# tabahi/WebSpeechAnalyzer

Measured on AMD Instinct MI355X. Metric: 53-feat frames/sec, higher is better.
Workload: dtype f32 front end / f64 tracker; 1 GPU; 1024 clips x 10 s @16 kHz mono per GPU, 1024-pt FFT, 25 ms hop, Segment Features (level 5); parallelism=1 GPU, batches_in_flight=6, streams=3

## Files before the change

### webspeechanalyzer_amd/csrc/tracker.hip

```cpp
#include <type_traits>
#include "wsa_internal.hpp"
#include "jsmath_device.hpp"
#include "wave_ops.hpp"
#include "tracker_score.hpp"
#include "tracker_features.hpp"

#ifdef WSA_TUNING
#define WSA_TUNE(bits_) (p.dbg & (bits_))
#else
#define WSA_TUNE(bits_) false
#endif

namespace wsa {

constexpr int MAXC = 64;
constexpr int AC_MAX = 320;
constexpr int PAIR_AC = 64;
constexpr int PAIR_GSZ = 4384;
constexpr int QUAD_AC = 38;
constexpr int QUAD_GSZ = 2496;
constexpr int AC_FAST = 140;

struct Ws {
    int32_t *tr_len, *tr_slot, *tr_rank;
// ... 108 lines not shown
        t.item++;
        const uint2 e = p.order[idx];
        t.clip = e.x; t.seg = e.y;
    }
    else if (DEAL == DEAL_GROUPS) {
        t.total = p.counters[p.order_cnt];
        const uint32_t npairs = (t.total + (uint32_t)NGR - 1u) / (uint32_t)NGR, W_ = gridDim.x, r = t.item;
        if ((uint64_t)r * W_ >= npairs) return SPAN_DONE;
        t.item++;
        t.group = (uint64_t)r * W_ + ((r & 1u) ? W_ - 1u - blockIdx.x : blockIdx.x);
        if (t.group >= npairs) return SPAN_SKIP;
    }
    else if (p.order) {
        const uint32_t total = p.counters[p.order_cnt], W_ = gridDim.x, r = t.item;
        if ((uint64_t)r * W_ >= total) return SPAN_DONE;
        t.item++;
        const uint64_t idx = (uint64_t)r * W_ + ((r & 1u) ? W_ - 1u - blockIdx.x : blockIdx.x);
        if (idx >= total) return SPAN_SKIP;
        const uint2 e = p.order[idx];
        t.clip = e.x; t.seg = e.y;
    } else {
        t.seg = t.item / p.n_clips; t.clip = t.item - t.seg * p.n_clips;
        if (t.seg >= p.counters[0]) return SPAN_DONE;
        t.item += gridDim.x;
        if (t.seg >= p.seg_count[t.clip]) return SPAN_SKIP;
    }
    return SPAN_TAKE;
}

}
#include "tracker_finalize.hpp"
#include "tracker_one.hpp"
#include "tracker_group.hpp"
namespace wsa {

template <int AC, bool RAW>
__device__ __forceinline__ void one_span_body(const TrParams& p) {
    const OneLds<AC> L = carve_lds<AC>();
    const int lane = threadIdx.x;
    SpanState sp;
    sp.W = carve_ws(p.ws + (uint64_t)blockIdx.x * p.ws_stride, p.tcap, p.pcap, p.fcap, RAW ? p.pcap : 0, nullptr);
    sp.gen = 0; sp.aev_stride = p.fcap + 2;
    for (int d = lane; d < p.fcap + 2; d += 64) sp.W.d_gen[d] = 0;
    wsync();
    SpanTurn t{p.order ? 0u : blockIdx.x};
    for (;;) {
        const int turn = next_span<DEAL_SPANS>(p, t);
        if (turn == SPAN_DONE) break;
        if (turn == SPAN_SKIP) continue;
        sp.begin(p, t.clip, (int)t.seg); sp.load_segment(p, true); sp.gen++;
        const unsigned long long tk0 = (WSA_TUNE(DBG_CYCLES)) ? __builtin_readcyclecounter() : 0ull;
        track_span<AC, RAW>(p, sp, L, lane);
        const unsigned long long tk1 = (WSA_TUNE(DBG_CYCLES)) ? __builtin_readcyclecounter() : 0ull;
        finish_span<AC, RAW, false>(p, sp, L, lane);
        trace_span_cycles(p, sp, lane, tk0, tk1);
        if (sp.overflow && lane == 0) atomicOr(&p.shared[1], sp.act_overflow && AC < AC_MAX ? 2u : 1u);
        wsync();
    }
}
template <int AC, bool RAW>
__device__ __forceinline__ void stream_body(const TrParams& p) {
    const OneLds<AC> L = carve_lds<AC>();
    const int lane = threadIdx.x;
    SpanState sp;
    sp.W = carve_ws(p.ws + (uint64_t)blockIdx.x * p.ws_stride, p.tcap, p.pcap, p.fcap, RAW ? p.pcap : 0, nullptr);
    sp.aev_stride = p.fcap + 2;
    wsync();
    sp.begin(p, blockIdx.x, 0);
    const unsigned long long tk0 = (WSA_TUNE(DBG_CYCLES)) ? __builtin_readcyclecounter() : 0ull;
    track_stream<AC, RAW>(p, sp, L, lane);
    trace_span_cycles(p, sp, lane, tk0, tk0);
    if (sp.overflow && lane == 0) atomicOr(&p.shared[1], 1u);
    wsync();
}
template <int AC, int GW, int SPLIT>
__device__ __forceinline__ void group_body(const TrParams& p) {
    const OneLds<AC, GW == 16> L = carve_lds<AC, GW == 16>();
    const int lane = threadIdx.x;
    SpanState sp;
    sp.gen = 0; sp.aev_stride = p.fcap + 2;
    if (!SPLIT) for (int h = 0; h < 2; h++) {
        const Ws Wh = carve_ws(p.ws + ((uint64_t)blockIdx.x * 2 + h) * p.ws_stride, p.tcap, p.pcap, p.fcap, 0, nullptr);
        for (int d = lane; d < p.fcap + 2; d += 64) Wh.d_gen[d] = 0;
    }
    wsync();
    SpanTurn t{p.order ? 0u : blockIdx.x};
    for (;;) {
        const int turn = next_span<DEAL_GROUPS, 64 / GW>(p, t);
        if (turn == SPAN_DONE) break;
        if (turn == SPAN_SKIP) continue;
        sp.gen++;
        track_group<AC, GW, SPLIT>(p, sp, L, lane, t);
    }
}
template <int AC>
__device__ __forceinline__ void finalize_body(const TrParams& p) {
    const OneLds<AC> L = carve_lds<AC>();
    const int lane = threadIdx.x;
    SpanState sp;
    wsync();
    SpanTurn t{p.order ? 0u : blockIdx.x};
    for (;;) {
        if (next_span<DEAL_FINALIZE>(p, t) == SPAN_DONE) break;
        sp.begin(p, t.clip, (int)t.seg); sp.load_segment(p, true);
        finalize_from_header<AC>(p, sp, L, lane);
    }
}

__global__ __launch_bounds__(64) __attribute__((amdgpu_waves_per_eu(4, 4))) void tracker_kernel_fast(TrParams p) { one_span_body<AC_FAST, false>(p); }
__global__ __launch_bounds__(64) __attribute__((amdgpu_waves_per_eu(3, 4))) void tracker_kernel_pair(TrParams p) {
    __builtin_amdgcn_s_setprio(3);
    group_body<AC_FAST, 32, 0>(p);
}
__global__ __launch_bounds__(64) __attribute__((amdgpu_waves_per_eu(4, 4))) void tracker_kernel_pair_acc(TrParams p) {
    __builtin_amdgcn_s_setprio(3);
    group_body<AC_FAST, 32, 1>(p);
}
__global__ __launch_bounds__(64) __attribute__((amdgpu_waves_per_eu(4, 4))) void tracker_kernel_quad_acc(TrParams p) {
    __builtin_amdgcn_s_setprio(3);
    group_body<AC_FAST, 16, 1>(p);
}
__global__ __launch_bounds__(64) __attribute__((amdgpu_waves_per_eu(4, 4))) void tracker_kernel_finalize(TrParams p) {
    __builtin_amdgcn_s_setprio(3);
    finalize_body<AC_FAST>(p);
}
__global__ __launch_bounds__(64) void tracker_kernel_full(TrParams p) { one_span_body<AC_MAX, false>(p); }
__global__ __launch_bounds__(64) void tracker_kernel_raw(TrParams p) { one_span_body<AC_MAX, true>(p); }
__global__ __launch_bounds__(64) void tracker_kernel_stream(TrParams p) { stream_body<AC_MAX, false>(p); }
__global__ __launch_bounds__(64) void tracker_kernel_stream_raw(TrParams p) { stream_body<AC_MAX, true>(p); }

constexpr int ORDER_T = 256;
__global__ __launch_bounds__(ORDER_T) void span_order_kernel(const uint32_t* hist, const uint2* key, const uint32_t* seg_count, uint32_t n_clips, int seg_cap, uint2* order, uint32_t* counters) {
    __shared__ uint32_t offs[SPAN_BUCKETS], part[ORDER_T];
    const int tid = threadIdx.x;
    constexpr int PER = SPAN_BUCKETS / ORDER_T;
    uint32_t mine[PER], sum = 0;
#pragma unroll
    for (int q = 0; q < PER; q++) { mine[q] = hist[tid * PER + q]; sum += mine[q]; }
    part[tid] = sum;
    __syncthreads();
    for (int d = 1; d < ORDER_T; d <<= 1) {
        const uint32_t add = tid >= d ? part[tid - d] : 0u;
        __syncthreads();
        part[tid] += add;
        __syncthreads();
    }
    uint32_t run = part[tid] - sum;
#pragma unroll
    for (int q = 0; q < PER; q++) { offs[tid * PER + q] = run; run += mine[q]; }
    if (blockIdx.x == 0 && tid == ORDER_T - 1) counters[1] = part[tid];
    __syncthreads();
    const uint32_t clip = blockIdx.x * ORDER_T + tid;
    if (clip >= n_clips) return;
    const uint32_t ns = seg_count[clip];
    for (uint32_t k = 0; k < ns; k++) {
        const uint2 e = key[(uint64_t)clip * seg_cap + k];
        order[offs[e.x] + e.y] = make_uint2(clip, k);
    }
}

void launch_span_order(const TrParams& p, uint32_t* span_hist, const uint2* span_key, uint2* order, uint32_t* counters, hipStream_t s) {
    if (p.n_clips == 0) return;
    hipLaunchKernelGGL(span_order_kernel, dim3((p.n_clips + ORDER_T - 1) / ORDER_T), dim3(ORDER_T), 0, s, span_hist, span_key, p.seg_count, p.n_clips, p.seg_cap, order, counters);
}

void launch_tracker_stream(const TrParams& p, uint32_t n_streams, hipStream_t s) {
    if (n_streams == 0) return;
    static_assert(AC_MAX == TR_ACT_MAX, "the streams' saved active table is sized for the full variant");
    if (p.level == 3) hipLaunchKernelGGL(tracker_kernel_stream_raw, dim3(n_streams), dim3(64), 0, s, p);
    else hipLaunchKernelGGL(tracker_kernel_stream, dim3(n_streams), dim3(64), 0, s, p);
}

void launch_tracker(const TrParams& p, int n_waves, bool full_table, bool pair, hipStream_t s) {
    if (n_waves <= 0) return;
    if (p.level == 3) hipLaunchKernelGGL(tracker_kernel_raw, dim3(n_waves), dim3(64), 0, s, p);
    else if (full_table) hipLaunchKernelGGL(tracker_kernel_full, dim3(n_waves), dim3(64), 0, s, p);
    else if (pair && p.order && p.redo && (!p.trace || (p.dbg & DBG_CYCLES))) {
        if (p.pool && p.span_hdr) {
            if (p.quad) hipLaunchKernelGGL(tracker_kernel_quad_acc, dim3(p.quad_waves > 0 ? p.quad_waves : n_waves), dim3(64), 0, s, p);
            else hipLaunchKernelGGL(tracker_kernel_pair_acc, dim3(n_waves), dim3(64), 0, s, p);
            hipLaunchKernelGGL(tracker_kernel_finalize, dim3(p.fin_waves > 0 ? p.fin_waves : 2 * n_waves), dim3(64), 0, s, p);
        }
        else hipLaunchKernelGGL(tracker_kernel_pair, dim3(n_waves), dim3(64), 0, s, p);
        TrParams r = p; r.order = p.redo; r.order_cnt = 2; r.pool = nullptr; r.span_hdr = nullptr;
        const int redo_waves = p.quad ? 1024 : 128;
        hipLaunchKernelGGL(tracker_kernel_fast, dim3(n_waves < redo_waves ? n_waves : redo_waves), dim3(64), 0, s, r);
    }
    else hipLaunchKernelGGL(tracker_kernel_fast, dim3(n_waves), dim3(64), 0, s, p);
}

__global__ void compact_count_kernel(CompactParams p) {
    const uint32_t c = blockIdx.x * blockDim.x + threadIdx.x;
    if (c >= p.n_clips) return;
    const uint32_t ns = p.seg_count[c];
    const int32_t* sg = p.seg_i + (uint64_t)c * p.seg_cap * 8;
    uint32_t r = 0;
    for (uint32_t k = 0; k < ns; k++) if (sg[8 * k + SEG_FLAG] >= 0) r += (uint32_t)sg[8 * k + SEG_NROWS];
    p.clip_row_off[c] = r;
}
constexpr int CSCAN_T = 1024;
template <bool COUNT>
__global__ __launch_bounds__(CSCAN_T) void compact_scan_kernel(CompactParams p) {
    __shared__ uint32_t s_rows[CSCAN_T], s_segs[CSCAN_T];
    const int tid = threadIdx.x;
    const uint32_t per = (p.n_clips + CSCAN_T - 1) / CSCAN_T;
    const uint32_t c0 = min(p.n_clips, tid * per), c1 = min(p.n_clips, c0 + per);
    uint32_t rs = 0, ss = 0;
    for (uint32_t c = c0; c < c1; c++) {
        if (COUNT) {
            const uint32_t ns = p.seg_count[c];
            const int32_t* sg = p.seg_i + (uint64_t)c * p.seg_cap * 8;
            uint32_t r = 0;
            for (uint32_t k = 0; k < ns; k++) if (sg[8 * k + SEG_FLAG] >= 0) r += (uint32_t)sg[8 * k + SEG_NROWS];
            p.clip_row_off[c] = r;
        }
        ss += p.seg_count[c]; rs += p.clip_row_off[c];
    }
    s_rows[tid] = rs; s_segs[tid] = ss;
    __syncthreads();
    for (int d = 1; d < CSCAN_T; d <<= 1) {
        const uint32_t ar_ = tid >= d ? s_rows[tid - d] : 0u, as_ = tid >= d ? s_segs[tid - d] : 0u;
        __syncthreads();
        s_rows[tid] += ar_; s_segs[tid] += as_;
        __syncthreads();
    }
    if (tid == CSCAN_T - 1) {
        p.totals[0] = s_rows[tid]; p.totals[1] = s_segs[tid];
        p.clip_row_off[p.n_clips] = s_rows[tid]; p.clip_seg_off[p.n_clips] = s_segs[tid];
    }
    uint32_t ar = s_rows[tid] - rs, as = s_segs[tid] - ss;
    for (uint32_t c = c0; c < c1; c++) {
        const uint32_t r = p.clip_row_off[c];
        p.clip_row_off[c] = ar; p.clip_seg_off[c] = as; as += p.seg_count[c]; ar += r;
    }
// ... 90 lines not shown
```

### webspeechanalyzer_amd/csrc/tracker_finalize.hpp

```cpp
#pragma once

namespace wsa {

__device__ __forceinline__ long long take_rows(const TrParams& p, SpanState& sp, int lane, int n) {
    uint32_t r0 = 0;
    if (lane == 0) r0 = atomicAdd(&p.clip_rows[sp.clip], (uint32_t)n);
    r0 = (uint32_t)read_lane_i32((int)r0, 0);
    if ((uint64_t)r0 + (uint32_t)n > p.row_cap) { sp.overflow = true; return -1; }
    return (long long)sp.clip * p.row_cap + r0;
}
template <typename Clear>
__device__ __forceinline__ int qualify_tracks(const Ws& W, int n_tr, int lane, double* qmb, int32_t* qt, Clear&& clear) {
    int nq = 0;
    for (int base = 0; base < n_tr; base += 64) {
        const int t = base + lane;
        bool q = false; double mb = 0;
        if (t < n_tr) {
            clear(t);
            const int tl = W.tr_len[t]; const double sb = W.tr_sumEbin[t], se = W.tr_sumE[t];
            if (tl >= 2) { mb = sb / se; q = mb >= 7; }
        }
        const uint64_t mask = __ballot(q);
        if (q) { const int pos = nq + __popcll(mask & lanemask_lt(lane)); qmb[pos] = mb; qt[pos] = t; }
        nq += __popcll(mask);
// ... 40 lines not shown
template <typename Part>
__device__ __forceinline__ bool files_past_the_end(const SpanState& sp, int lane, bool by_index, Part&& takes_part) {
    bool bad = false;
    for (int base = sp.len; base <= (by_index ? sp.c_ci + 1 : -1); base += 64) {
        const int d = base + lane;
        if (d <= sp.c_ci + 1 && sp.W.d_gen[d] == sp.gen)
            for (int q = sp.W.d_p0[d]; q < sp.W.d_p1[d]; q++) if (takes_part(q)) bad = true;
    }
    if (sp.stale_d >= sp.len && lane == 0)
        for (int q = 0; q < sp.stale_p1; q++) if (takes_part(q)) bad = true;
    return bad;
}
template <typename Key, typename KeyOf, typename Point>
__device__ __forceinline__ void straighten_select(const TrParams& p, const SpanState& sp, int lane, float* fr, float* smv, KeyOf&& key_of, Point&& point) {
    for (int base = 0; base < ((WSA_TUNE(DBG_NO_STRAIGHTEN)) ? 0 : sp.len); base += 64) {
        const int d = base + lane;
        if (d < sp.len) {
            float f9[9];
#pragma unroll
            for (int q = 0; q < 9; q++) f9[q] = 0.f;
            float sm = 0.f;
            const int a1 = (sp.stale_d == d) ? sp.stale_p1 : 0;
            const int dg = sp.W.d_gen[d], dp0 = sp.W.d_p0[d], dp1 = sp.W.d_p1[d];
            const bool has_main = dg == sp.gen;
            const int b0 = has_main ? dp0 : 0, b1 = has_main ? dp1 : 0;
            Key last_key = -1;
            for (;;) {
                Key best_key = sizeof(Key) == 4 ? (Key)0x7fffffff : (Key)0x7fffffffffffffffLL; int best_q = -1;
                for (int part = 0; part < 2; part++) {
                    const int q0 = part ? b0 : 0, q1 = part ? b1 : a1;
                    for (int q = q0; q < q1; q++) {
                        const Key key = key_of(q);
                        if (key > last_key && key < best_key) { best_key = key; best_q = q; }
                    }
                }
                if (best_q < 0) break;
                last_key = best_key;
                int l; double f, wd, E;
                point(best_q, l, f, wd, E);
                const float cur = l == 0 ? f9[0] : (l == 1 ? f9[3] : f9[6]);
                if ((double)cur > sp.floor_ && (double)cur < f && l < 2) l++;
                const float ff = (float)f, Ef = (float)E, wf = (float)wd;
                if (l == 0) { f9[0] = ff; f9[1] = Ef; f9[2] = wf; }
                else if (l == 1) { f9[3] = ff; f9[4] = Ef; f9[5] = wf; }
                else { f9[6] = ff; f9[7] = Ef; f9[8] = wf; }
                sm = (float)((double)sm + E);
            }
#pragma unroll
            for (int q = 0; q < 9; q++) fr[9 * d + q] = f9[q];
            smv[d] = sm;
        }
    }
}
template <bool LANES, typename Feat>
__device__ __forceinline__ void write_rows(const TrParams& p, SpanState& sp, int lane, const float* fr, const float* smv, Feat&& features) {
    if (p.formants && (p.level == 4 || p.level == 10)) {
        for (int q = lane; q < 9 * sp.len; q += 64) { const int d = q / 9; p.formants[((uint64_t)sp.foff + (((uint32_t)sp.start + (uint32_t)d) & p.ring_mask)) * 9 + (uint32_t)(q - 9 * d)] = fr[q]; }
        if (p.sums) { for (int q = lane; q < sp.len; q += 64) p.sums[(uint64_t)sp.foff + (((uint32_t)sp.start + (uint32_t)q) & p.ring_mask)] = smv[q]; }
    }
    double accS, accC; sp.totals(accS, accC);
    const double cs = accC / accS;
    const double lg_ctx = jsm::log10(sp.ctx_max);
    if (p.level == 4 || p.level == 5) {
        const long long r0 = take_rows(p, sp, lane, 1);
        if (r0 < 0) return;
        double* x = p.row_feat + (uint64_t)r0 * WSA_NFEAT;
        if (WSA_TUNE(DBG_CYCLES)) sp.ph[2] = __builtin_readcyclecounter();
        if (p.level == 5) {
            if (!(WSA_TUNE(DBG_NO_FEATURES))) features(fr, sp.len, x);
            if (WSA_TUNE(DBG_CYCLES)) sp.ph[3] = __builtin_readcyclecounter();
            if (lane == 0) { x[0] = sp.len; x[1] = sqrt((double)sp.len); x[2] = cs; x[3] = lg_ctx; x[4] = sp.floor_; }
        } else if (lane < WSA_NFEAT) x[lane] = 0;
        if (lane == 0) {
            int32_t* m = p.row_meta + (uint64_t)r0 * 8;
            m[0] = (int32_t)sp.clip; m[1] = 0; m[2] = 0; m[3] = 0; m[4] = sp.my_seg; m[5] = 0; m[6] = sp.start; m[7] = sp.len;
            sp.sg[SEG_FLAG] = 1; sp.sg[SEG_NROWS] = 1; sp.sg[SEG_ROW0] = (int32_t)r0;
        }
        return;
    }
    int nsyl = 0, my_si = 0, my_sl = 0;
    {
        int si = -1, cc = 0, uu = 0;
        for (int base = 0; base < sp.len; base += 64) {
            const int dd = base + lane;
            const float smq = dd < sp.len ? smv[dd] : 0.f;
            const int lim = min(64, sp.len - base);
            for (int j = 0; j < lim; j++) {
                const int e2 = base + j;
                const double v = __builtin_bit_cast(float, read_lane_i32(__builtin_bit_cast(int, smq), j));
                if (v > sp.floor_) { cc = 0; uu++; if (si < 0) si = e2; } else cc++;
                if ((uu > 20 && cc > 0) || (uu > 10 && cc > 1) || (uu > 0 && cc > 4) || (e2 >= sp.len - 1 && uu > 4)) {
                    const int t = e2 - cc;
                    if (t - si > 1) {
                        if (LANES && nsyl < 64) { if (lane == nsyl) { my_si = si; my_sl = t - si; } }
                        else if (lane == 0) { sp.W.q_idx[2 * nsyl] = si; sp.W.q_idx[2 * nsyl + 1] = t - si; }
                        nsyl++;
                        si = -1; uu = 0;
                    }
                }
            }
        }
    }
    wsync();
    long long r0 = 0;
    if (nsyl > 0) { r0 = take_rows(p, sp, lane, nsyl); if (r0 < 0) return; }
    for (int k = 0; k < nsyl; k++) {
        const int si = LANES && k < 64 ? read_lane_i32(my_si, k) : sp.W.q_idx[2 * k], sl = LANES && k < 64 ? read_lane_i32(my_sl, k) : sp.W.q_idx[2 * k + 1];
        double* x = p.row_feat + (uint64_t)(r0 + k) * WSA_NFEAT;
        if (p.level == 13) {
            if (!(WSA_TUNE(DBG_NO_FEATURES))) features(fr + 9 * si, sl, x);
            if (lane == 0) { x[0] = sl; x[1] = sqrt((double)sl); x[2] = cs; x[3] = lg_ctx; x[4] = sp.floor_; }
        } else if (lane < WSA_NFEAT) x[lane] = 0;
        if (lane == 0) {
            int32_t* m = p.row_meta + (uint64_t)(r0 + k) * 8;
            m[0] = (int32_t)sp.clip; m[1] = 0; m[2] = si; m[3] = sl; m[4] = sp.my_seg; m[5] = k; m[6] = sp.start + si; m[7] = sl;
        }
    }
    if (lane == 0) { sp.sg[SEG_FLAG] = nsyl > 0 ? 1 : 0; sp.sg[SEG_NROWS] = nsyl; sp.sg[SEG_ROW0] = (int32_t)r0; }
}
template <int AC, bool G>
__device__ __forceinline__ bool finalize_lds(const TrParams& p, SpanState& sp, const OneLds<AC>& L, int lane) {
    constexpr int BIG = OneLds<AC>::BYTES;
    const int off_u = (int)align16((size_t)2 * sp.n_tr);
    const int rank_bytes = 16 * sp.n_tr, fr_bytes = G ? 0 : (int)align16((size_t)40 * sp.len);
    const int off_pt = off_u + fr_bytes;
    const bool pe_lds = !G && off_pt + 12 * sp.n_pt <= BIG;
    const int ppb = pe_lds ? 12 : 4;
    if (sp.n_tr > 8000 || sp.n_pt > 60000 || off_u + rank_bytes > BIG || off_pt + ppb * sp.n_pt > BIG || off_pt + FEAT_SCRATCH * 8 > BIG) return false;
    int16_t* const trk_key = reinterpret_cast<int16_t*>(L.big);
    double* const qmb = reinterpret_cast<double*>(L.big + off_u);
    int32_t* const qt = reinterpret_cast<int32_t*>(L.big + off_u + 8 * sp.n_tr);
    int32_t* const srt = qt + sp.n_tr;
    float* const fr = G ? sp.W.fr : reinterpret_cast<float*>(L.big + off_u);
    float* const smv = G ? sp.W.sm1 : fr + 9 * sp.len;
    double* const pE = reinterpret_cast<double*>(L.big + off_pt);
    uint32_t* const pkb = reinterpret_cast<uint32_t*>(L.big + off_pt + (pe_lds ? 8 * sp.n_pt : 0));
    auto energy_of = [&](int q) __attribute__((always_inline)) -> double { return pe_lds ? pE[q] : reinterpret_cast<const double*>(sp.W.pt + q)[1]; };
    if (WSA_TUNE(DBG_CYCLES)) sp.ph[0] = sp.ph[1] = sp.ph[2] = sp.ph[3] = __builtin_readcyclecounter();
    const int nq = qualify_tracks(sp.W, sp.n_tr, lane, qmb, qt, [&](int t) __attribute__((always_inline)) { trk_key[t] = -1; });
    wsync();
    rank_tracks(nq, qmb, lane, [&](int rank, int qi) __attribute__((always_inline)) { srt[rank] = qi; });
    wsync();
    const int n_part = assign_slots(nq, qmb, qt, srt, lane, [&](int t, int key) __attribute__((always_inline)) { trk_key[t] = (int16_t)key; });
    wsync();
    const int off_tbl = (int)align16((size_t)off_pt + (size_t)ppb * (size_t)sp.n_pt);
    const int tbl_bytes = 4 * (sp.len + 1) + 2 * (sp.len + 1) * n_part;
    const bool use_tbl = !G && n_part <= 32 && sp.c_ci + 1 < 0x7fff && sp.stale_d < 0x7fff && off_tbl + tbl_bytes <= BIG && !(p.dbg & DBG_SELECT_LOOP);
    uint32_t* const tblm = reinterpret_cast<uint32_t*>(L.big + off_tbl);
    uint16_t* const tbl = reinterpret_cast<uint16_t*>(tblm + sp.len + 1);
    if (use_tbl) for (int q = lane; q <= sp.len; q += 64) tblm[q] = 0u;
    wsync();
    bool bad = false;
    {
        int4 nxt4 = lane < sp.n_pt ? sp.W.pt[lane] : make_int4(0, 0, 0, 0);
        for (int q = lane; q < sp.n_pt; q += 64) {
            const int4 rec4 = nxt4;
            if (q + 64 < sp.n_pt) nxt4 = sp.W.pt[q + 64];
            const int key = trk_key[rec4.x];
            if (pe_lds) pE[q] = __hiloint2double(rec4.w, rec4.z);
            pkb[q] = ((uint32_t)rec4.y & 0x1ffffu) | ((key < 0 ? 0x7fffu : (uint32_t)key) << 17);
            if (use_tbl && key >= 0) {
                const int d = (int)((uint32_t)rec4.y >> 17);
                if (d >= sp.len) bad = true;
                else {
                    const int row = (q < sp.stale_p1 && sp.stale_d >= 0) ? sp.len : d;
                    tbl[row * n_part + (key >> 2)] = (uint16_t)(q + 1);
                    atomicOr(&tblm[row], 1u << (key >> 2));
                }
            }
        }
    }
    wsync();
    if (WSA_TUNE(DBG_CYCLES)) sp.ph[0] = __builtin_readcyclecounter();
    if (files_past_the_end(sp, lane, !use_tbl, [&](int q) __attribute__((always_inline)) { return (pkb[q] >> 17) != 0x7fffu; })) bad = true;
    if (__ballot(bad) != 0ull) { if (lane == 0) { sp.sg[SEG_FLAG] = -1; sp.sg[SEG_NROWS] = 0; } return true; }
    if (use_tbl) {
        const uint32_t stale_m = tblm[sp.len];
        float thr_f;
        { const double t0 = sp.floor_ < 0 ? 0.0 : floor(sp.floor_) + 1.0; thr_f = (float)(t0 > 256.0 ? 256.0 : t0); }
        for (int base = 0; base < ((WSA_TUNE(DBG_NO_STRAIGHTEN)) ? 0 : sp.len); base += 64) {
            const int d = base + lane;
            float* const row = fr + 9 * (d < sp.len ? d : 0);
            if (d < sp.len) {
#pragma unroll
                for (int q = 0; q < 9; q++) row[q] = 0.f;
            }
            float sm = 0.f;
            auto apply = [&](int q) __attribute__((always_inline)) {
                const uint32_t w = pkb[q];
                int l = (int)((w >> 17) & 3u);
                const double E = energy_of(q);
                const float ff = (float)(w & 0xffu), cur = row[3 * l];
                if (cur >= thr_f && cur < ff && l < 2) l++;
                row[3 * l] = ff; row[3 * l + 1] = (float)E; row[3 * l + 2] = (float)((w >> 8) & 0x1ffu);
                sm = (float)((double)sm + E);
            };
            const uint32_t m_main = d < sp.len ? tblm[d] : 0u, m_st = (d < sp.len && d == sp.stale_d) ? stale_m : 0u;
            uint32_t mm = m_main | m_st;
            while (mm) {
                const int r = __ffs((int)mm) - 1; mm &= mm - 1u;
                if ((m_st >> r) & 1u) apply((int)tbl[sp.len * n_part + r] - 1);
                if ((m_main >> r) & 1u) apply((int)tbl[d * n_part + r] - 1);
            }
            if (d < sp.len) smv[d] = sm;
        }
    } else
    straighten_select<int>(p, sp, lane, fr, smv,
        [&](int q) __attribute__((always_inline)) -> int { const uint32_t w = pkb[q]; return (w >> 17) == 0x7fffu ? -1 : (int)(((w >> 19) << 16) | (uint32_t)q); },
        [&](int q, int& l, double& f, double& wd, double& E) __attribute__((always_inline)) {
            const uint32_t w = pkb[q];
            l = (int)((w >> 17) & 3u); f = w & 0xffu; wd = (w >> 8) & 0x1ffu; E = energy_of(q);
        });
    wsync();
    if (WSA_TUNE(DBG_CYCLES)) sp.ph[1] = __builtin_readcyclecounter();
    double* const red = reinterpret_cast<double*>(L.big + off_pt);
    write_rows<true>(p, sp, lane, fr, smv, [&](const float* f, int n, double* x) __attribute__((always_inline)) {
        formant_features_lds(f, n, sp.ctx_max, x, lane, red, !G && n <= 15 && !(p.dbg & DBG_NO_PACKED_COLUMNS), G || (p.dbg & DBG_EVENTS_BLOCK) != 0);
    });
    return true;
}
template <int AC>
__device__ __forceinline__ void finalize_generic(const TrParams& p, SpanState& sp, const OneLds<AC>& L, int lane) {
    constexpr int FRCAP = OneLds<AC>::FRCAP;
    if (WSA_TUNE(DBG_CYCLES)) sp.ph[0] = sp.ph[1] = sp.ph[2] = sp.ph[3] = __builtin_readcyclecounter();
    const int nq = qualify_tracks(sp.W, sp.n_tr, lane, sp.W.q_mb, sp.W.q_idx, [&](int t) __attribute__((always_inline)) { sp.W.tr_slot[t] = -1; });
    wsync();
    const bool q_lds = nq <= AC;
    double* qmb = sp.W.q_mb; int32_t* qidx = sp.W.q_idx; int32_t* sorted = sp.W.sorted;
    if (q_lds) {
        for (int qi = lane; qi < nq; qi += 64) { L.f_qmb[qi] = sp.W.q_mb[qi]; L.f_qidx[qi] = sp.W.q_idx[qi]; }
        qmb = L.f_qmb; qidx = L.f_qidx; sorted = L.f_sorted;
        wsync();
    }
    rank_tracks(nq, qmb, lane, [&](int rank, int qi) __attribute__((always_inline)) { sorted[rank] = qi; });
    wsync();
    assign_slots(nq, qmb, qidx, sorted, lane, [&](int t, int key) __attribute__((always_inline)) { sp.W.tr_slot[t] = key; });
    wsync();
    {
        int t_nxt = lane < sp.n_pt ? sp.W.pt[lane].x : 0;
        for (int q = lane; q < sp.n_pt; q += 64) {
            const int t = t_nxt;
            if (q + 64 < sp.n_pt) t_nxt = sp.W.pt[q + 64].x;
            sp.W.pt_key[q] = sp.W.tr_slot[t];
        }
    }
    wsync();
    if (WSA_TUNE(DBG_CYCLES)) sp.ph[0] = __builtin_readcyclecounter();
    if (__ballot(files_past_the_end(sp, lane, true, [&](int q) __attribute__((always_inline)) { return sp.W.pt_key[q] >= 0; })) != 0ull) { if (lane == 0) { sp.sg[SEG_FLAG] = -1; sp.sg[SEG_NROWS] = 0; } return; }
    float* const fr = sp.len <= FRCAP ? L.f_fr : sp.W.fr;
    float* const smv_ = sp.len <= FRCAP ? L.f_sm : sp.W.sm1;
    auto features = [&](const float* f, int a, double* x) __attribute__((always_inline)) {
        if (sp.len > FRCAP && a <= FEAT_LDS_MAX) formant_features_lds(f, a, sp.ctx_max, x, lane, reinterpret_cast<double*>(L.big), false, true);
        else formant_features_wave(f, a, sp.ctx_max, x, sp.W.Aev, sp.aev_stride, lane);
    };
    straighten_select<long long>(p, sp, lane, fr, smv_,
        [&](int q) __attribute__((always_inline)) -> long long { const int pk = sp.W.pt_key[q]; return pk < 0 ? -1LL : (long long)(pk >> 2) * (long long)(p.pcap + 1) + q; },
        [&](int q, int& l, double& f, double& wd, double& E) __attribute__((always_inline)) {
            l = sp.W.pt_key[q] & 3;
            const int4 rec4 = sp.W.pt[q];
            f = rec4.y & 0xff; wd = (rec4.y >> 8) & 0x1ff; E = __hiloint2double(rec4.w, rec4.z);
        });
    wsync();
    if (WSA_TUNE(DBG_CYCLES)) sp.ph[1] = __builtin_readcyclecounter();
    write_rows<false>(p, sp, lane, fr, smv_, features);
}
__device__ __forceinline__ void export_raw_tracks(const TrParams& p, SpanState& sp, int lane, bool ring) {
    const int nq = qualify_tracks(sp.W, sp.n_tr, lane, sp.W.q_mb, sp.W.q_idx, [](int) __attribute__((always_inline)) {});
    wsync();
    const uint64_t pbase = (uint64_t)sp.foff * MAXC;
    const uint64_t pmask = ring ? (uint64_t)(p.ring_mask + 1u) * MAXC - 1ull : ~0ull;
    const uint64_t poff = (ring ? (uint64_t)((uint32_t)sp.sg[SEG_FBEGIN] & p.ring_mask) : (uint64_t)sp.f_begin) * MAXC;
    const uint64_t pool0 = pbase + poff;
    auto slot = [&](uint64_t q) __attribute__((always_inline)) -> uint64_t { return pbase + ((poff + q) & pmask); };
    rank_tracks(nq, sp.W.q_mb, lane, [&](int rank, int qi) __attribute__((always_inline)) { p.trk_rank[slot((uint64_t)rank)] = sp.W.q_idx[qi]; });
    for (int q = lane; q < sp.n_pt; q += 64) { int4 v = sp.W.pt[q]; v.y &= 0x1ffff; p.trk_pts[2 * slot((uint64_t)q)] = v; p.trk_pts[2 * slot((uint64_t)q) + 1] = sp.W.ptx[q]; }
    if (lane == 0) {
        int32_t* ts = p.trk_seg + ((uint64_t)sp.clip * p.seg_cap + sp.my_seg) * 4;
        ts[0] = (int32_t)(pool0 & 0xffffffffu); ts[1] = sp.n_pt; ts[2] = nq; ts[3] = (int32_t)(pool0 >> 32);
    }
}
template <int AC, bool RAW, bool THIRD>
__device__ __forceinline__ void finish_span(const TrParams& p, SpanState& sp, const OneLds<AC>& L, int lane, bool ring = false) {
    for (int j = lane; j < sp.n_act; j += 64) { const int gi = L.a_gid[j]; sp.W.tr_len[gi] = L.a_len[j]; sp.W.tr_sumE[gi] = L.a_sumE[j]; sp.W.tr_sumEbin[gi] = L.a_sumEbin[j]; }
    wsync();
    if constexpr (RAW) export_raw_tracks(p, sp, lane, ring);
    else if (!(WSA_TUNE(DBG_NO_FINALIZE))) {
        if (!(p.dbg & DBG_GENERIC_FINALIZE)) {
            if (finalize_lds<AC, false>(p, sp, L, lane)) return;
            if constexpr (THIRD) { if (!(p.dbg & DBG_NO_THIRD_FORM) && finalize_lds<AC, true>(p, sp, L, lane)) return; }
        }
        finalize_generic<AC>(p, sp, L, lane);
    }
}
template <int AC>
__device__ __forceinline__ void finalize_from_header(const TrParams& p, SpanState& sp, const OneLds<AC>& L, int lane) {
    const double* hd = p.span_hdr + ((uint64_t)sp.clip * p.seg_cap + (uint32_t)sp.my_seg) * 8;
    const double h0 = hd[0], h1 = hd[1], h2 = hd[2], h3 = hd[3], h4 = hd[4], h5 = hd[5], h6 = hd[6];
    const int flag = (int)h6;
    if (flag == 0) return;
    if (flag & 2) { if (lane == 0) atomicOr(&p.shared[1], 1u); return; }
    const int F = (int)(sp.f_end - sp.f_begin);
    sp.W = carve_ws(p.pool + (uint64_t)(sp.foff + sp.f_begin) * p.pool_bpf, MAXC * F, MAXC * F, F, 0, nullptr);
    sp.aev_stride = F + 2;
    sp.n_tr = (int)h0; sp.n_pt = (int)h1; sp.n_act = 0; sp.stale_d = (int)h2; sp.stale_p1 = (int)h3;
    sp.accG = h4; sp.accL = lane == 0 ? h5 : 0.0;
    sp.gen = 1;
    const unsigned long long tf0 = WSA_TUNE(DBG_CYCLES) ? __builtin_readcyclecounter() : 0ull;
    finish_span<AC, false, true>(p, sp, L, lane);
    if (WSA_TUNE(DBG_CYCLES) && lane == 0 && p.trace) {
        double* tr = p.trace + (uint64_t)atomicAdd(&p.shared[0], 1u) * 12;
        tr[0] = 0; tr[1] = (double)(__builtin_readcyclecounter() - tf0); tr[2] = sp.len; tr[3] = F; tr[4] = sp.n_tr; tr[5] = sp.n_pt; tr[6] = blockIdx.x;
        tr[7] = (double)(sp.ph[0] - tf0); tr[8] = (double)(sp.ph[1] - sp.ph[0]); tr[9] = (double)(sp.ph[2] - sp.ph[1]); tr[10] = (double)(sp.ph[3] - sp.ph[2]);
    }
    if (sp.overflow && lane == 0) atomicOr(&p.shared[1], 1u);
    wsync();
}

}
```

### webspeechanalyzer_amd/csrc/tracker_group.hpp

```cpp
#pragma once

namespace wsa {

template <int GW>
struct GroupLds {
    static constexpr int ACG = GW == 32 ? PAIR_AC : QUAD_AC, NGR = 64 / GW, GSZ = GW == 32 ? PAIR_GSZ : QUAD_GSZ;
    static_assert(GSZ % 16 == 0 && GSZ >= ACG * 48 + GW * 40 + 24 && (ACG * 24) % 8 == 0 && (ACG * 48 + GW * 20) % 8 == 0, "group layout fits its share of the block");
    double *t_vel, *t_sumE, *t_sumEbin; uint32_t* t_mmask; int32_t *t_lf, *t_len, *t_gid; uint32_t *t_bins, *t_amp;
    uint32_t *q_pk, *q_amp, *q_plo, *q_phi, *q_hi;
    unsigned long long* q_best; int32_t *q_asg, *q_prj, *q_pro;
    uint32_t* q_map;
    __device__ __forceinline__ GroupLds(unsigned char* big, int g) {
        unsigned char* const gb = big + g * GSZ;
        t_vel = reinterpret_cast<double*>(gb); t_sumE = t_vel + ACG; t_sumEbin = t_sumE + ACG;
        t_mmask = reinterpret_cast<uint32_t*>(t_sumEbin + ACG);
        t_lf = reinterpret_cast<int32_t*>(t_mmask + ACG); t_len = t_lf + ACG; t_gid = t_len + ACG;
        t_bins = reinterpret_cast<uint32_t*>(t_gid + ACG); t_amp = t_bins + ACG;
        q_pk = t_amp + ACG; q_amp = q_pk + GW; q_plo = q_amp + GW; q_phi = q_plo + GW; q_hi = q_phi + GW;
        q_best = reinterpret_cast<unsigned long long*>(q_hi + GW);
        q_asg = reinterpret_cast<int32_t*>(q_best + GW); q_prj = q_asg + GW; q_pro = q_prj + GW;
        q_map = reinterpret_cast<uint32_t*>(q_pro + GW);
    }
};
struct GroupState {
// ... 222 lines not shown
                    G.t_lf[j] = nfile; G.t_len[j] = 1; G.t_gid[j] = t; G.t_bins[j] = (uint32_t)pk_l; G.t_amp[j] = pamp;
                    G.t_vel[j] = 0; G.t_sumE[j] = be; G.t_sumEbin[j] = be * pk_l;
                    gs.W.pt[q] = make_int4(t, pk_l | ((pk_s - pk_i + 1) << 8) | (min(nfile, 0x7fff) << 17), __double2loint(be), __double2hiint(be));
                }
                if (grow) { gs.ntr += nnew; gs.npt += nnew; gs.nact += nnew; }
                if (on) {
                    if (rst) { gs.stale_d = nfile; gs.stale_p1 = gs.npt; }
                    else if (gl == 0 && nfile < gs.fcap + 2) { gs.W.d_p0[nfile] = p_begin; gs.W.d_p1[nfile] = gs.npt; gs.W.d_gen[nfile] = SPLIT ? 1 : gen; }
                }
                wsync();
                gs.clk.lap(WSA_TUNE(DBG_CYCLES), 4);
            }
        }
        h0 = h1; h1 = h2; c0 = c1;
    }
    return nsteps;
}
template <int GW>
__device__ __forceinline__ void write_span_headers(const TrParams& p, const GroupState& gs, int lane) {
    constexpr int NGR = 64 / GW;
    const int g = lane / GW, gl = lane % GW;
    double cg[NGR];
#pragma unroll
    for (int q = 0; q < NGR; q++) cg[q] = g == q ? gs.accL : 0.0;
    wave_sums_f64(cg);
    double c_mine = cg[0];
#pragma unroll
    for (int q = 1; q < NGR; q++) c_mine = g == q ? cg[q] : c_mine;
    if (gs.has && gl == 0) {
        if (gs.redo) { const uint32_t k = atomicAdd(p.redo_count, 1u); p.redo[k] = make_uint2(gs.clip, gs.seg); }
        double* hd = p.span_hdr + ((uint64_t)gs.clip * p.seg_cap + gs.seg) * 8;
        hd[0] = gs.ntr; hd[1] = gs.npt; hd[2] = gs.stale_d; hd[3] = gs.stale_p1; hd[4] = gs.accG; hd[5] = c_mine;
        hd[6] = gs.redo ? 0.0 : (gs.ovf ? 2.0 : 1.0);
    }
}
template <int AC>
__device__ __forceinline__ void finalize_pair(const TrParams& p, SpanState& sp, const GroupState& gs, const OneLds<AC>& L, int lane) {
    const int g = lane / 32;
    for (int h = 0; h < 2; h++) {
        const int src = h * 32;
        if (!read_lane_i32((int)gs.has, src)) continue;
        const uint32_t clip = (uint32_t)read_lane_i32((int)gs.clip, src), seg = (uint32_t)read_lane_i32((int)gs.seg, src);
        if (read_lane_i32((int)gs.redo, src)) {
            if (lane == 0) { const uint32_t k = atomicAdd(p.redo_count, 1u); p.redo[k] = make_uint2(clip, seg); }
            continue;
        }
        sp.begin(p, clip, (int)seg); sp.load_segment(p, true);
        sp.n_tr = read_lane_i32(gs.ntr, src); sp.n_pt = read_lane_i32(gs.npt, src); sp.n_act = 0;
        sp.stale_d = read_lane_i32(gs.stale_d, src); sp.stale_p1 = read_lane_i32(gs.stale_p1, src);
        sp.accG = read_lane_f64(gs.accG, src);
        sp.accL = g == h ? gs.accL : 0.0;
        sp.overflow = read_lane_i32((int)gs.ovf, src) != 0; sp.act_overflow = false;
        sp.W = carve_ws(p.ws + ((uint64_t)blockIdx.x * 2 + (uint32_t)h) * p.ws_stride, p.tcap, p.pcap, p.fcap, 0, nullptr);
        if (!sp.overflow) finish_span<AC, false, false>(p, sp, L, lane);
        if (sp.overflow && lane == 0) atomicOr(&p.shared[1], 1u);
        wsync();
    }
}
template <int AC, int GW, int SPLIT>
__device__ __forceinline__ void track_group(const TrParams& p, SpanState& sp, const OneLds<AC, GW == 16>& L, int lane, const SpanTurn& t) {
    static_assert(GW == 32 || (GW == 16 && SPLIT == 1), "four spans per wave only as the accumulate half of the split tracker");
    static_assert(GW <= GW_MAX, "the SPLIT kernels' span regions are sized for at most GW_MAX new tracks / points per frame (see tracker_pool_bpf)");
    static_assert(GroupLds<GW>::NGR * GroupLds<GW>::GSZ <= OneLds<AC, GW == 16>::BYTES, "the groups fit the block");
    const int gl = lane % GW;
    const GroupLds<GW> G(L.big, lane / GW);
    GroupState gs;
    group_begin<GW, SPLIT>(p, gs, G, lane, t);
    const unsigned long long ptk0 = WSA_TUNE(DBG_CYCLES) ? __builtin_readcyclecounter() : 0ull;
    const int nsteps = group_accumulate<GW, SPLIT>(p, gs, G, lane, sp.gen);
    const unsigned long long ptk1 = WSA_TUNE(DBG_CYCLES) ? __builtin_readcyclecounter() : 0ull;
    for (int j = gl; j < gs.nact; j += GW) { const int gi = G.t_gid[j]; gs.W.tr_len[gi] = G.t_len[j]; gs.W.tr_sumE[gi] = G.t_sumE[j]; gs.W.tr_sumEbin[gi] = G.t_sumEbin[j]; }
    wsync();
    if constexpr (SPLIT == 1) write_span_headers<GW>(p, gs, lane);
    else finalize_pair<AC>(p, sp, gs, L, lane);
    if (WSA_TUNE(DBG_CYCLES) && lane == 0 && p.trace) {
        double* tr = p.trace + (uint64_t)atomicAdd(&p.shared[0], 1u) * 12;
        tr[0] = (double)(ptk1 - ptk0); tr[1] = (double)(__builtin_readcyclecounter() - ptk1); tr[2] = nsteps; tr[3] = gs.pn_on; tr[4] = gs.pn_chunk2; tr[5] = gs.pn_pass; tr[6] = blockIdx.x;
        tr[7] = (double)gs.clk.cy[0]; tr[8] = (double)gs.clk.cy[1]; tr[9] = (double)gs.clk.cy[2]; tr[10] = (double)gs.clk.cy[3]; tr[11] = (double)gs.clk.cy[4];
    }
}

}
```

### webspeechanalyzer_amd/csrc/tracker_one.hpp

```cpp
#pragma once

namespace wsa {
struct Hdr { int info; double v, fl; uint4 h; };
struct Pre { int info; double v, fl, g; int n; uint32_t pk, amp, plo, phi, hi; };
__device__ __forceinline__ void load_hdr(const TrParams& p, const SpanState& sp, int vz, uint32_t f, Hdr& q) {
    const uint32_t fi = (min(f, sp.f_end - 1) & p.ring_mask) + (uint32_t)vz;
    q.info = p.fr_info[sp.foff + fi]; q.v = p.fr_v[sp.foff + fi]; q.fl = p.fr_fl[sp.foff + fi];
    q.h = p.rec.hdr[sp.foff + fi];
}
__device__ __forceinline__ void load_ent(const TrParams& p, const SpanState& sp, int lane, uint32_t f, const Hdr& h, Pre& q) {
    const int hy = read_first_lane_i32((int)h.h.y);
    q.info = f < sp.f_end ? read_first_lane_i32(h.info) : -1; q.v = read_first_lane_f64(h.v); q.fl = read_first_lane_f64(h.fl);
    q.g = (double)(hy & 0xff) * 4294967296.0 + (double)(uint32_t)read_first_lane_i32((int)h.h.x);
    q.n = (hy >> 8) & 0xff; q.pk = q.amp = q.plo = q.phi = q.hi = 0;
    if (q.info >= 0 && lane < q.n && !(WSA_TUNE(DBG_NO_ENTRIES))) {
        const uint32_t c = (uint32_t)read_first_lane_i32((int)h.h.w) + (uint32_t)lane;
        const uint4 e4 = p.rec.ent[c];
        q.amp = p.rec.amp[c]; q.pk = e4.x; q.plo = e4.y; q.phi = e4.z; q.hi = e4.w;
    }
}
template <int AC, bool RAW, typename Refill>
__device__ __forceinline__ void accumulate(const TrParams& p, SpanState& sp, const OneLds<AC>& L, int lane, const Pre& cur, Refill&& refill) {
    const int info = cur.info;
    if (!(info >= 0 && !(WSA_TUNE(DBG_NO_ACCUMULATE)))) { refill(); return; }
// ... 206 lines not shown
    if (sp.f_begin + 64 < sp.f_end) load_blk(sp.f_begin + 64, bn);
    Ent ring[PFD];
    #pragma unroll
    for (int k = 0; k < PFD; k++) request(k, ring[k]);
    for (uint32_t blk = sp.f_begin; blk < sp.f_end; blk += 64) {
      const int nb = (int)min(64u, sp.f_end - blk);
      for (int j0 = 0; j0 < nb; j0 += PFD) {
    #pragma unroll
        for (int k = 0; k < PFD; k++) {
          const int j = j0 + k;
          if (j >= nb) break;
          Pre cur;
          const int hy = read_lane_i32((int)bc.h.y, j);
          cur.info = read_lane_i32(bc.info, j); cur.v = read_lane_f64(bc.v, j); cur.fl = read_lane_f64(bc.fl, j);
          cur.g = (double)(hy & 0xff) * 4294967296.0 + (double)(uint32_t)read_lane_i32((int)bc.h.x, j);
          cur.n = (hy >> 8) & 0xff;
          cur.pk = ring[k].pk; cur.amp = ring[k].amp; cur.plo = ring[k].plo; cur.phi = ring[k].phi; cur.hi = ring[k].hi;
          accumulate<AC, RAW>(p, sp, L, lane, cur, [&]() __attribute__((always_inline)) { request(j + PFD, ring[k]); });
          if (p.trace && !(WSA_TUNE(DBG_CYCLES))) { double accS, accC; sp.totals(accS, accC); if (lane == 0) { double* tr = p.trace + ((uint64_t)sp.foff + blk + (uint32_t)j) * 12; tr[10] = accS; tr[11] = accC; } }
        }
      }
      bc = bn;
      if (blk + 128 < sp.f_end && !(WSA_TUNE(DBG_NO_PREFETCH))) load_blk(blk + 128, bn);
    }
}
template <int AC, bool RAW>
__device__ __forceinline__ void track_stream(const TrParams& p, SpanState& sp, const OneLds<AC>& L, int lane) {
    int vz; asm volatile("v_mov_b32 %0, 0" : "=v"(vz));
    int32_t* stt = p.st_state + (uint64_t)sp.clip * TR_STATE_WORDS;
    double* std_ = reinterpret_cast<double*>(stt + 8);
    sp.n_tr = stt[0]; sp.n_pt = stt[1]; sp.n_act = stt[2]; sp.stale_d = stt[3]; sp.stale_p1 = stt[4]; int my_span = stt[5]; sp.gen = stt[6];
    sp.accG = std_[0] + std_[1]; sp.accL = lane == 0 ? std_[1] : 0.0;
    char* ab = p.st_act + (uint64_t)sp.clip * TR_ACT_BYTES;
    double* const g_vel = reinterpret_cast<double*>(ab); double* const g_sumE = g_vel + AC; double* const g_sumEbin = g_sumE + AC;
    int32_t* const g_lf = reinterpret_cast<int32_t*>(g_sumEbin + AC); int32_t* const g_len = g_lf + AC; int32_t* const g_gid = g_len + AC;
    uint32_t* const g_bins = reinterpret_cast<uint32_t*>(g_gid + AC); uint32_t* const g_amp = g_bins + AC;
    for (int j = lane; j < sp.n_act; j += 64) {
        L.a_vel[j] = g_vel[j]; L.a_sumE[j] = g_sumE[j]; L.a_sumEbin[j] = g_sumEbin[j];
        L.a_last_frame[j] = g_lf[j]; L.a_len[j] = g_len[j]; L.a_gid[j] = g_gid[j]; L.a_bins[j] = g_bins[j]; L.a_amp[j] = g_amp[j];
    }
    wsync();
    auto clear_state = [&](int span) __attribute__((always_inline)) { sp.clear_tracks(); sp.gen++; my_span = span; };
    const uint32_t nfr = p.n_frames_step[sp.clip];
    const uint32_t fbase = (uint32_t)p.gate_state[(uint64_t)sp.clip * GATE_STATE] - nfr;
    const int nseg = (int)p.seg_count[sp.clip];
    sp.f_begin = fbase; sp.f_end = fbase + nfr;
    int ks = 0;
    auto close_segments = [&](uint32_t f_next, bool all) __attribute__((always_inline)) {
        while (ks < nseg) {
            int32_t* sgk = p.seg_i + ((uint64_t)sp.clip * p.seg_cap + ks) * 8;
            if (!all && (uint32_t)sgk[SEG_FEND] != f_next) break;
            if (sgk[SEG_FBEGIN] != my_span) clear_state(sgk[SEG_FBEGIN]);
            sp.my_seg = ks; sp.load_segment(p, false);
            finish_span<AC, RAW, false>(p, sp, L, lane, true);
            clear_state(-2);
            ks++;
        }
    };
    for (uint32_t f = fbase; f < fbase + nfr; f++) {
        Hdr h; load_hdr(p, sp, vz, f, h);
        Pre cur; load_ent(p, sp, lane, f, h, cur);
        if (cur.info >= 0) {
            const int span = p.fr_span[sp.foff + (f & p.ring_mask)];
            if (span != my_span) clear_state(span);
            accumulate<AC, RAW>(p, sp, L, lane, cur, [] {});
        }
        close_segments(f + 1, false);
    }
    close_segments(0, true);
    double accS, accC; sp.totals(accS, accC);
    if (lane == 0) { stt[0] = sp.n_tr; stt[1] = sp.n_pt; stt[2] = sp.n_act; stt[3] = sp.stale_d; stt[4] = sp.stale_p1; stt[5] = my_span; stt[6] = sp.gen; std_[0] = accS; std_[1] = accC; }
    for (int j = lane; j < sp.n_act; j += 64) {
        g_vel[j] = L.a_vel[j]; g_sumE[j] = L.a_sumE[j]; g_sumEbin[j] = L.a_sumEbin[j];
        g_lf[j] = L.a_last_frame[j]; g_len[j] = L.a_len[j]; g_gid[j] = L.a_gid[j]; g_bins[j] = L.a_bins[j]; g_amp[j] = L.a_amp[j];
    }
}

}
```

Before: 764.2 million frames/s.

## Specialize finalize kernel on level and outline declined-span fallback path

The finalize kernel is templated on the feature level so level checks fold at compile time, and the launcher picks an instantiation from p.level. The rare fallback (third LDS form or generic finalize) moves into a noinline function that reloads params from the kernarg pointer, keeping it out of the hot path's register allocation. Params are re-read each loop iteration through an opaque kernarg pointer to shorten live ranges. The intent is to lower VGPR/SGPR pressure and code size in the hot finalize kernel, at the cost of a real call with its overhead on declined spans.

```diff
diff --git a/webspeechanalyzer_amd/csrc/tracker.hip b/webspeechanalyzer_amd/csrc/tracker.hip
--- a/webspeechanalyzer_amd/csrc/tracker.hip
+++ b/webspeechanalyzer_amd/csrc/tracker.hip
@@ -184,7 +184,7 @@
         const unsigned long long tk0 = (WSA_TUNE(DBG_CYCLES)) ? __builtin_readcyclecounter() : 0ull;
         track_span<AC, RAW>(p, sp, L, lane);
         const unsigned long long tk1 = (WSA_TUNE(DBG_CYCLES)) ? __builtin_readcyclecounter() : 0ull;
-        finish_span<AC, RAW, false>(p, sp, L, lane);
+        finish_span<AC, RAW>(p, sp, L, lane);
         trace_span_cycles(p, sp, lane, tk0, tk1);
         if (sp.overflow && lane == 0) atomicOr(&p.shared[1], sp.act_overflow && AC < AC_MAX ? 2u : 1u);
         wsync();
@@ -225,17 +225,21 @@
         track_group<AC, GW, SPLIT>(p, sp, L, lane, t);
     }
 }
-template <int AC>
-__device__ __forceinline__ void finalize_body(const TrParams& p) {
+template <int AC, int LV>
+__device__ __forceinline__ void finalize_body(const TrParams& p0) {
     const OneLds<AC> L = carve_lds<AC>();
-    const int lane = threadIdx.x;
+    int lane = threadIdx.x;
     SpanState sp;
     wsync();
-    SpanTurn t{p.order ? 0u : blockIdx.x};
+    SpanTurn t{p0.order ? 0u : blockIdx.x};
     for (;;) {
+        asm volatile("" : "+v"(lane));
+        kernarg_ptr kargs = (kernarg_ptr)__builtin_amdgcn_kernarg_segment_ptr();
+        asm volatile("" : "+s"(kargs));
+        const TrParams& p = *(const TrParams*)kargs;
         if (next_span<DEAL_FINALIZE>(p, t) == SPAN_DONE) break;
         sp.begin(p, t.clip, (int)t.seg); sp.load_segment(p, true);
-        finalize_from_header<AC>(p, sp, L, lane);
+        finalize_from_header<AC, LV>(p, (const void*)kargs, sp, L, lane);
     }
 }
 
@@ -252,9 +256,10 @@
     __builtin_amdgcn_s_setprio(3);
     group_body<AC_FAST, 16, 1>(p);
 }
+template <int LV>
 __global__ __launch_bounds__(64) __attribute__((amdgpu_waves_per_eu(4, 4))) void tracker_kernel_finalize(TrParams p) {
     __builtin_amdgcn_s_setprio(3);
-    finalize_body<AC_FAST>(p);
+    finalize_body<AC_FAST, LV>(p);
 }
 __global__ __launch_bounds__(64) void tracker_kernel_full(TrParams p) { one_span_body<AC_MAX, false>(p); }
 __global__ __launch_bounds__(64) void tracker_kernel_raw(TrParams p) { one_span_body<AC_MAX, true>(p); }
@@ -311,7 +316,11 @@
         if (p.pool && p.span_hdr) {
             if (p.quad) hipLaunchKernelGGL(tracker_kernel_quad_acc, dim3(p.quad_waves > 0 ? p.quad_waves : n_waves), dim3(64), 0, s, p);
             else hipLaunchKernelGGL(tracker_kernel_pair_acc, dim3(n_waves), dim3(64), 0, s, p);
-            hipLaunchKernelGGL(tracker_kernel_finalize, dim3(p.fin_waves > 0 ? p.fin_waves : 2 * n_waves), dim3(64), 0, s, p);
+            const dim3 fin_grid(p.fin_waves > 0 ? p.fin_waves : 2 * n_waves);
+            if (p.level == 5) hipLaunchKernelGGL(tracker_kernel_finalize<5>, fin_grid, dim3(64), 0, s, p);
+            else if (p.level == 13) hipLaunchKernelGGL(tracker_kernel_finalize<13>, fin_grid, dim3(64), 0, s, p);
+            else if (p.level == 4) hipLaunchKernelGGL(tracker_kernel_finalize<4>, fin_grid, dim3(64), 0, s, p);
+            else hipLaunchKernelGGL(tracker_kernel_finalize<10>, fin_grid, dim3(64), 0, s, p);
         }
         else hipLaunchKernelGGL(tracker_kernel_pair, dim3(n_waves), dim3(64), 0, s, p);
         TrParams r = p; r.order = p.redo; r.order_cnt = 2; r.pool = nullptr; r.span_hdr = nullptr;
diff --git a/webspeechanalyzer_amd/csrc/tracker_finalize.hpp b/webspeechanalyzer_amd/csrc/tracker_finalize.hpp
--- a/webspeechanalyzer_amd/csrc/tracker_finalize.hpp
+++ b/webspeechanalyzer_amd/csrc/tracker_finalize.hpp
@@ -116,21 +116,23 @@
         }
     }
 }
-template <bool LANES, typename Feat>
+template <int LV> __device__ __forceinline__ int level_of(const TrParams& p) { return LV ? LV : p.level; }
+template <bool LANES, int LV, typename Feat>
 __device__ __forceinline__ void write_rows(const TrParams& p, SpanState& sp, int lane, const float* fr, const float* smv, Feat&& features) {
-    if (p.formants && (p.level == 4 || p.level == 10)) {
+    const int level = level_of<LV>(p);
+    if (p.formants && (level == 4 || level == 10)) {
         for (int q = lane; q < 9 * sp.len; q += 64) { const int d = q / 9; p.formants[((uint64_t)sp.foff + (((uint32_t)sp.start + (uint32_t)d) & p.ring_mask)) * 9 + (uint32_t)(q - 9 * d)] = fr[q]; }
         if (p.sums) { for (int q = lane; q < sp.len; q += 64) p.sums[(uint64_t)sp.foff + (((uint32_t)sp.start + (uint32_t)q) & p.ring_mask)] = smv[q]; }
     }
     double accS, accC; sp.totals(accS, accC);
     const double cs = accC / accS;
     const double lg_ctx = jsm::log10(sp.ctx_max);
-    if (p.level == 4 || p.level == 5) {
+    if (level == 4 || level == 5) {
         const long long r0 = take_rows(p, sp, lane, 1);
         if (r0 < 0) return;
         double* x = p.row_feat + (uint64_t)r0 * WSA_NFEAT;
         if (WSA_TUNE(DBG_CYCLES)) sp.ph[2] = __builtin_readcyclecounter();
-        if (p.level == 5) {
+        if (level == 5) {
             if (!(WSA_TUNE(DBG_NO_FEATURES))) features(fr, sp.len, x);
             if (WSA_TUNE(DBG_CYCLES)) sp.ph[3] = __builtin_readcyclecounter();
             if (lane == 0) { x[0] = sp.len; x[1] = sqrt((double)sp.len); x[2] = cs; x[3] = lg_ctx; x[4] = sp.floor_; }
@@ -171,7 +173,7 @@
     for (int k = 0; k < nsyl; k++) {
         const int si = LANES && k < 64 ? read_lane_i32(my_si, k) : sp.W.q_idx[2 * k], sl = LANES && k < 64 ? read_lane_i32(my_sl, k) : sp.W.q_idx[2 * k + 1];
         double* x = p.row_feat + (uint64_t)(r0 + k) * WSA_NFEAT;
-        if (p.level == 13) {
+        if (level == 13) {
             if (!(WSA_TUNE(DBG_NO_FEATURES))) features(fr + 9 * si, sl, x);
             if (lane == 0) { x[0] = sl; x[1] = sqrt((double)sl); x[2] = cs; x[3] = lg_ctx; x[4] = sp.floor_; }
         } else if (lane < WSA_NFEAT) x[lane] = 0;
@@ -182,7 +184,7 @@
     }
     if (lane == 0) { sp.sg[SEG_FLAG] = nsyl > 0 ? 1 : 0; sp.sg[SEG_NROWS] = nsyl; sp.sg[SEG_ROW0] = (int32_t)r0; }
 }
-template <int AC, bool G>
+template <int AC, bool G, int LV>
 __device__ __forceinline__ bool finalize_lds(const TrParams& p, SpanState& sp, const OneLds<AC>& L, int lane) {
     constexpr int BIG = OneLds<AC>::BYTES;
     const int off_u = (int)align16((size_t)2 * sp.n_tr);
@@ -278,12 +280,12 @@
     wsync();
     if (WSA_TUNE(DBG_CYCLES)) sp.ph[1] = __builtin_readcyclecounter();
     double* const red = reinterpret_cast<double*>(L.big + off_pt);
-    write_rows<true>(p, sp, lane, fr, smv, [&](const float* f, int n, double* x) __attribute__((always_inline)) {
+    write_rows<true, LV>(p, sp, lane, fr, smv, [&](const float* f, int n, double* x) __attribute__((always_inline)) {
         formant_features_lds(f, n, sp.ctx_max, x, lane, red, !G && n <= 15 && !(p.dbg & DBG_NO_PACKED_COLUMNS), G || (p.dbg & DBG_EVENTS_BLOCK) != 0);
     });
     return true;
 }
-template <int AC>
+template <int AC, int LV>
 __device__ __forceinline__ void finalize_generic(const TrParams& p, SpanState& sp, const OneLds<AC>& L, int lane) {
     constexpr int FRCAP = OneLds<AC>::FRCAP;
     if (WSA_TUNE(DBG_CYCLES)) sp.ph[0] = sp.ph[1] = sp.ph[2] = sp.ph[3] = __builtin_readcyclecounter();
@@ -326,7 +328,7 @@
         });
     wsync();
     if (WSA_TUNE(DBG_CYCLES)) sp.ph[1] = __builtin_readcyclecounter();
-    write_rows<false>(p, sp, lane, fr, smv_, features);
+    write_rows<false, LV>(p, sp, lane, fr, smv_, features);
 }
 __device__ __forceinline__ void export_raw_tracks(const TrParams& p, SpanState& sp, int lane, bool ring) {
     const int nq = qualify_tracks(sp.W, sp.n_tr, lane, sp.W.q_mb, sp.W.q_idx, [](int) __attribute__((always_inline)) {});
@@ -343,41 +345,64 @@
         ts[0] = (int32_t)(pool0 & 0xffffffffu); ts[1] = sp.n_pt; ts[2] = nq; ts[3] = (int32_t)(pool0 >> 32);
     }
 }
-template <int AC, bool RAW, bool THIRD>
+template <int AC, bool RAW, int LV = 0>
 __device__ __forceinline__ void finish_span(const TrParams& p, SpanState& sp, const OneLds<AC>& L, int lane, bool ring = false) {
     for (int j = lane; j < sp.n_act; j += 64) { const int gi = L.a_gid[j]; sp.W.tr_len[gi] = L.a_len[j]; sp.W.tr_sumE[gi] = L.a_sumE[j]; sp.W.tr_sumEbin[gi] = L.a_sumEbin[j]; }
     wsync();
     if constexpr (RAW) export_raw_tracks(p, sp, lane, ring);
     else if (!(WSA_TUNE(DBG_NO_FINALIZE))) {
-        if (!(p.dbg & DBG_GENERIC_FINALIZE)) {
-            if (finalize_lds<AC, false>(p, sp, L, lane)) return;
-            if constexpr (THIRD) { if (!(p.dbg & DBG_NO_THIRD_FORM) && finalize_lds<AC, true>(p, sp, L, lane)) return; }
-        }
-        finalize_generic<AC>(p, sp, L, lane);
-    }
-}
-template <int AC>
-__device__ __forceinline__ void finalize_from_header(const TrParams& p, SpanState& sp, const OneLds<AC>& L, int lane) {
+        if (!(p.dbg & DBG_GENERIC_FINALIZE) && finalize_lds<AC, false, LV>(p, sp, L, lane)) return;
+        finalize_generic<AC, LV>(p, sp, L, lane);
+    }
+}
+__device__ __forceinline__ bool span_from_header(const TrParams& p, SpanState& sp, int lane) {
     const double* hd = p.span_hdr + ((uint64_t)sp.clip * p.seg_cap + (uint32_t)sp.my_seg) * 8;
     const double h0 = hd[0], h1 = hd[1], h2 = hd[2], h3 = hd[3], h4 = hd[4], h5 = hd[5], h6 = hd[6];
     const int flag = (int)h6;
-    if (flag == 0) return;
-    if (flag & 2) { if (lane == 0) atomicOr(&p.shared[1], 1u); return; }
+    if (flag == 0) return false;
+    if (flag & 2) { if (lane == 0) atomicOr(&p.shared[1], 1u); return false; }
     const int F = (int)(sp.f_end - sp.f_begin);
     sp.W = carve_ws(p.pool + (uint64_t)(sp.foff + sp.f_begin) * p.pool_bpf, MAXC * F, MAXC * F, F, 0, nullptr);
     sp.aev_stride = F + 2;
     sp.n_tr = (int)h0; sp.n_pt = (int)h1; sp.n_act = 0; sp.stale_d = (int)h2; sp.stale_p1 = (int)h3;
     sp.accG = h4; sp.accL = lane == 0 ? h5 : 0.0;
     sp.gen = 1;
-    const unsigned long long tf0 = WSA_TUNE(DBG_CYCLES) ? __builtin_readcyclecounter() : 0ull;
-    finish_span<AC, false, true>(p, sp, L, lane);
+    return true;
+}
+__device__ __forceinline__ void span_finalized(const TrParams& p, SpanState& sp, int lane, unsigned long long tf0) {
     if (WSA_TUNE(DBG_CYCLES) && lane == 0 && p.trace) {
         double* tr = p.trace + (uint64_t)atomicAdd(&p.shared[0], 1u) * 12;
-        tr[0] = 0; tr[1] = (double)(__builtin_readcyclecounter() - tf0); tr[2] = sp.len; tr[3] = F; tr[4] = sp.n_tr; tr[5] = sp.n_pt; tr[6] = blockIdx.x;
+        tr[0] = 0; tr[1] = (double)(__builtin_readcyclecounter() - tf0); tr[2] = sp.len; tr[3] = (int)(sp.f_end - sp.f_begin); tr[4] = sp.n_tr; tr[5] = sp.n_pt; tr[6] = blockIdx.x;
         tr[7] = (double)(sp.ph[0] - tf0); tr[8] = (double)(sp.ph[1] - sp.ph[0]); tr[9] = (double)(sp.ph[2] - sp.ph[1]); tr[10] = (double)(sp.ph[3] - sp.ph[2]);
     }
     if (sp.overflow && lane == 0) atomicOr(&p.shared[1], 1u);
     wsync();
 }
+typedef __attribute__((address_space(4))) const void* kernarg_ptr;
+template <int AC>
+__device__ __attribute__((noinline)) void finalize_declined_span(const void* kargs, uint32_t clip, int seg, unsigned char* lds) {
+    const uint64_t ka = (uint64_t)kargs;
+    const uint64_t ka_u = ((uint64_t)(uint32_t)__builtin_amdgcn_readfirstlane((int)(ka >> 32)) << 32) | (uint32_t)__builtin_amdgcn_readfirstlane((int)(uint32_t)ka);
+    const TrParams& p = *(const TrParams*)(kernarg_ptr)ka_u;
+    typedef __attribute__((address_space(3))) unsigned char lds_uc;
+    const OneLds<AC> L((unsigned char*)(lds_uc*)lds);
+    const int lane = threadIdx.x;
+    SpanState sp;
+    sp.begin(p, (uint32_t)__builtin_amdgcn_readfirstlane((int)clip), __builtin_amdgcn_readfirstlane(seg)); sp.load_segment(p, true);
+    if (!span_from_header(p, sp, lane)) return;
+    const unsigned long long tf0 = WSA_TUNE(DBG_CYCLES) ? __builtin_readcyclecounter() : 0ull;
+    if ((p.dbg & (DBG_GENERIC_FINALIZE | DBG_NO_THIRD_FORM)) || !finalize_lds<AC, true, 0>(p, sp, L, lane)) finalize_generic<AC, 0>(p, sp, L, lane);
+    span_finalized(p, sp, lane, tf0);
+}
+template <int AC, int LV>
+__device__ __forceinline__ void finalize_from_header(const TrParams& p, const void* kargs, SpanState& sp, const OneLds<AC>& L, int lane) {
+    if (!span_from_header(p, sp, lane)) return;
+    const unsigned long long tf0 = WSA_TUNE(DBG_CYCLES) ? __builtin_readcyclecounter() : 0ull;
+    if (!(WSA_TUNE(DBG_NO_FINALIZE))) {
+        const bool done = !(p.dbg & DBG_GENERIC_FINALIZE) && finalize_lds<AC, false, LV>(p, sp, L, lane);
+        if (__builtin_expect(!done, 0)) { finalize_declined_span<AC>(kargs, sp.clip, sp.my_seg, L.big); return; }
+    }
+    span_finalized(p, sp, lane, tf0);
+}
 
 }
diff --git a/webspeechanalyzer_amd/csrc/tracker_group.hpp b/webspeechanalyzer_amd/csrc/tracker_group.hpp
--- a/webspeechanalyzer_amd/csrc/tracker_group.hpp
+++ b/webspeechanalyzer_amd/csrc/tracker_group.hpp
@@ -298,7 +298,7 @@
         sp.accL = g == h ? gs.accL : 0.0;
         sp.overflow = read_lane_i32((int)gs.ovf, src) != 0; sp.act_overflow = false;
         sp.W = carve_ws(p.ws + ((uint64_t)blockIdx.x * 2 + (uint32_t)h) * p.ws_stride, p.tcap, p.pcap, p.fcap, 0, nullptr);
-        if (!sp.overflow) finish_span<AC, false, false>(p, sp, L, lane);
+        if (!sp.overflow) finish_span<AC, false>(p, sp, L, lane);
         if (sp.overflow && lane == 0) atomicOr(&p.shared[1], 1u);
         wsync();
     }
diff --git a/webspeechanalyzer_amd/csrc/tracker_one.hpp b/webspeechanalyzer_amd/csrc/tracker_one.hpp
--- a/webspeechanalyzer_amd/csrc/tracker_one.hpp
+++ b/webspeechanalyzer_amd/csrc/tracker_one.hpp
@@ -282,7 +282,7 @@
             if (!all && (uint32_t)sgk[SEG_FEND] != f_next) break;
             if (sgk[SEG_FBEGIN] != my_span) clear_state(sgk[SEG_FBEGIN]);
             sp.my_seg = ks; sp.load_segment(p, false);
-            finish_span<AC, RAW, false>(p, sp, L, lane, true);
+            finish_span<AC, RAW>(p, sp, L, lane, true);
             clear_state(-2);
             ks++;
         }
```

Measured after the change: 768.4 million frames/s (median of 6 runs). Within noise of the previous version (+0.5%).
